# iris1997jiatong/I-DCCRN-VAE

Measured on AMD Instinct MI355X. Metric: 4s@16kHz utterances/sec fwd+SI-SNR, DCCRN-CL, 1/2/4/8 MI355X vs host CPU, higher is better.
Workload: dtype f32; 1 GPU; supervised DCCRN-CL forward(train=False) + final_ete_loss (weights 0/0/1); batch_per_gpu=64, utterance=4 s @ 16 kHz (64000 samples, 641 frames), parallelism=replicas x1, streams=1, input=resident in HBM

## Files before the change

i-dccrn-vae_amd/csrc/cgemm.hpp:

```cpp
#pragma once
#include "common.hpp"

#ifndef IDV_WAVES_PER_SIMD
#define IDV_WAVES_PER_SIMD 1
#endif

enum { IDV_CONV = 0, IDV_TCONV = 1, IDV_PW = 2 };

struct CgemmArgs {
    const float* x0;
    const float* x1;
    int C0, C1;
    int Fin, Fout;
    int J, Jp, Tp;
    int Jp1, x1_div;
    const float* wfrag;
    const float* bias;
    const float* slope;
    float* out;
    int M;
    int Mtiles;
    int cplx_rows;
    int Cout;
    int tshift;
    int t_valid;
    double* stats;
    int stats_rep;
    int ldo;
    int nB;
    int jtiles, ftiles, mblocks;
    int map_ft;
    long long lo_off0, lo_off1;
    void* out_img;
    long long out_lo_off;
};
#define IDV_IMG_ZSLOT (-8)

typedef __bf16 idv_bf16x2 __attribute__((ext_vector_type(2)));
__device__ __forceinline__ unsigned idv_pack_bf16(float a, float b) {
    idv_bf16x2 v = {(__bf16)a, (__bf16)b};
    return __builtin_bit_cast(unsigned, v);
}

template <int MODE, int FO_T>
struct CgemmGeom {
    static constexpr int KF = (MODE == IDV_PW) ? 1 : 5;
    static constexpr int FR = (MODE == IDV_CONV) ? 2 * FO_T + 3 : (MODE == IDV_TCONV ? FO_T + 2 : 1);
    static constexpr int ROWS = (MODE == IDV_TCONV) ? 2 * FO_T : FO_T;
};

struct CgemmFlatCols {
    static constexpr bool FLAT = true;
    __device__ __forceinline__ int in_col(const CgemmArgs&, int v) const { return v; }
    __device__ __forceinline__ void out_pos(const CgemmArgs& a, int v, int& b, int& tp) const {
        b = v / a.Tp;
        tp = v - b * a.Tp;
    }
    __device__ __forceinline__ void store(float* p, float y) const { *p = y; }
};
struct CgemmTimeChunkCols {
    static constexpr bool FLAT = false;
    int t0, steps;
    __device__ __forceinline__ int in_col(const CgemmArgs& a, int v) const {
        const int b = v / steps;
        return b * a.Tp + 1 + t0 + (v - b * steps);
    }
    __device__ __forceinline__ void out_pos(const CgemmArgs&, int v, int& b, int& tp) const {
        b = v / steps;
        tp = 1 + t0 + (v - b * steps);
    }
    __device__ __forceinline__ void store(float* p, float y) const { __hip_atomic_store(p, y, __ATOMIC_RELAXED, __HIP_MEMORY_SCOPE_AGENT); }
};

template <int MODE, int WM, int WN, int MT_W, int FO_T, int JC_W, int CCK, bool SWAP, bool STATS, bool VEC, class CM>
__device__ __forceinline__ void cgemm_tile(const CgemmArgs& a, float* smem, const int jt, const int ft, const int mblk, const CM cm) {
#define CGEMM_BODY_TILE_GIVEN
#include "cgemm_body.hpp"
#undef CGEMM_BODY_TILE_GIVEN
}

template <int MODE, int WM, int WN, int MT_W, int FO_T, int JC_W, int CCK, bool SWAP, bool STATS, bool VEC>
__global__ __launch_bounds__(WM* WN * 64, IDV_WAVES_PER_SIMD) void cgemm_kernel(const CgemmArgs a) {
    extern __shared__ __attribute__((aligned(16))) float smem[];
    using CM = CgemmFlatCols;
    const CM cm{};
#include "cgemm_body.hpp"
}
```

i-dccrn-vae_amd/csrc/cgemm_body.hpp:

```cpp
    using G = CgemmGeom<MODE, FO_T>;
    static_assert(CM::FLAT || (MODE == IDV_PW && SWAP && !VEC), "mapped columns: scalar staging of the point-wise SWAP form");
    constexpr int NT = WM * WN * 64;
    constexpr int KF = G::KF, FR = G::FR, ROWS = G::ROWS;
    constexpr int JT = 32 * JC_W * WN;
    constexpr int PS = VEC ? JT + 8 : JT + 2;
    constexpr int COL0 = VEC ? 4 : 1;
    constexpr int NE = CCK * FR * PS;
    constexpr int NLD = VEC ? 1 : (NE + NT - 1) / NT;
    constexpr int PS4 = PS / 4;
    constexpr int NV = CCK * FR * PS4;
    constexpr int NLD4 = VEC ? (NV + NT - 1) / NT : 1;
    static_assert(!VEC || NLD4 <= 8, "ok-mask holds 8 slots x 4 bits");
    constexpr int NCOL = ROWS * JC_W;
    constexpr int KSC = (MODE == IDV_PW) ? CCK / 2 : CCK * KF;
    static_assert(MODE != IDV_PW || (CCK % 2 == 0), "PW chunks are plane pairs");

    const int tid = threadIdx.x;
    const int lane = tid & 63;
    const int wave = __builtin_amdgcn_readfirstlane(tid >> 6);
    const int wm = wave / WN, wn = wave % WN;
#ifndef CGEMM_BODY_TILE_GIVEN

    const int MB = a.mblocks, FTn = a.ftiles;
    const int bid = blockIdx.x;
// ... 185 lines not shown

    constexpr int UNITS = (MODE == IDV_PW) ? CCK / 2 : CCK;
    const int bcol = wn * (JC_W * 32) + (lane & 31) + ((MODE == IDV_PW) ? COL0 : (lane >> 5) + COL0 + a.tshift);
    auto load_b = [&](const float* P, int u, float (&dst)[FR][JC_W]) {
#pragma unroll
        for (int fr = 0; fr < FR; ++fr)
#pragma unroll
            for (int jc = 0; jc < JC_W; ++jc) {
                if (MODE == IDV_PW)
                    dst[fr][jc] = P[(2 * u + (lane >> 5)) * PS + bcol + jc * 32];
                else
                    dst[fr][jc] = P[(u * FR + fr) * PS + bcol + jc * 32];
            }
    };

    stage_load(0);
    load_a(0, a_cur);
    stage_store(smem, 0);
#pragma unroll
    for (int ks = 0; ks < KSC; ++ks)
#pragma unroll
        for (int i = 0; i < MT_W; ++i) asm volatile("" : "+v"(a_cur[ks][i]));
    __syncthreads();

    for (int chunk = 0; chunk < nchunk; ++chunk) {
        const float* P = smem + (chunk & 1) * NE;
        const int nxt = (chunk + 1 < nchunk) ? chunk + 1 : chunk;
        float b_cur[FR][JC_W], b_nxt[FR][JC_W];
        load_b(P, 0, b_cur);
#pragma unroll
        for (int u = 0; u < UNITS; ++u) {
            if (u + 1 < UNITS) load_b(P, u + 1, b_nxt);
            __builtin_amdgcn_sched_barrier(0);
            if constexpr (CM::FLAT) {
                if (u == 0) {
                    stage_load(nxt);
                    load_a(nxt, a_nxt);
                }
            } else {
                constexpr int SPU = (2 * NLD + UNITS - 1) / UNITS;
#pragma unroll
                for (int q = 0; q < SPU; ++q)
                    if (u * SPU + q < NLD) stage_load_slot(nxt, u * SPU + q);
                static_assert(MODE != IDV_PW || KSC == UNITS, "one k-step per unit");
            }
            if (u == UNITS - 1) stage_store(smem + ((chunk + 1) & 1) * NE, nxt);
#pragma unroll
            for (int kf = 0; kf < KF; ++kf) {
                const int ks = (MODE == IDV_PW) ? u : u * KF + kf;
#pragma unroll
                for (int rt = 0; rt < ROWS; ++rt) {
                    int fr;
                    if (MODE == IDV_CONV) {
                        fr = 2 * rt + kf;
                    } else if (MODE == IDV_TCONV) {
                        if ((rt & 1) != (kf & 1)) continue;
                        fr = (rt >> 1) + 2 - (kf >> 1);
                    } else {
                        fr = 0;
                    }
#pragma unroll
                    for (int jc = 0; jc < JC_W; ++jc)
#pragma unroll
                        for (int i = 0; i < MT_W; ++i) {
                            if (SWAP)
                                acc[i][rt * JC_W + jc] = __builtin_amdgcn_mfma_f32_32x32x2f32(b_cur[fr][jc], a_cur[ks][i], acc[i][rt * JC_W + jc], 0, 0, 0);
                            else
                                acc[i][rt * JC_W + jc] = __builtin_amdgcn_mfma_f32_32x32x2f32(a_cur[ks][i], b_cur[fr][jc], acc[i][rt * JC_W + jc], 0, 0, 0);
                        }
                }
            }
            if constexpr (!CM::FLAT) load_a_ks(nxt, u, a_cur);
            if (u + 1 < UNITS) {
#pragma unroll
                for (int fr = 0; fr < FR; ++fr)
#pragma unroll
                    for (int jc = 0; jc < JC_W; ++jc) b_cur[fr][jc] = b_nxt[fr][jc];
            }
        }
        if constexpr (CM::FLAT) {
#pragma unroll
            for (int ks = 0; ks < KSC; ++ks)
#pragma unroll
                for (int i = 0; i < MT_W; ++i) a_cur[ks][i] = a_nxt[ks][i];
        }
        __syncthreads();
    }

    if (a.out_img && blockIdx.x == 0 && tid < 2) {
        unsigned short* z = (unsigned short*)a.out_img + IDV_IMG_ZSLOT * 8 + (tid ? a.out_lo_off : 0);
        *(uint4*)z = make_uint4(0u, 0u, 0u, 0u);
    }
    const float slope = a.slope ? *a.slope : 1.0f;
    const bool has_act = a.slope != nullptr;
    const int half = lane >> 5, l31 = lane & 31;

    if (!SWAP) {
#pragma unroll
        for (int i = 0; i < MT_W; ++i) {
            const int mt = mt0 + i;
            float bia[16];
#pragma unroll
            for (int r = 0; r < 16; ++r) {
                const int m = mt * 32 + (r & 3) + 8 * (r >> 2) + 4 * half;
                bia[r] = a.bias[m];
            }
            float st[STATS ? 8 : 1][5];
            if (STATS) {
#pragma unroll
                for (int q = 0; q < 8; ++q)
#pragma unroll
                    for (int s = 0; s < 5; ++s) st[q][s] = 0.f;
            }
// ... 96 lines not shown
```

i-dccrn-vae_amd/csrc/lstm.hip:

```cpp
#include "common.hpp"
#include "../../include/idccrn_hip.h"

namespace {

struct RecArgs {
    const float* g;
    long long g_run_z;
    long long g_run_s;
    int ldg;
    const float* whh;
    float* hout;
    int H, B, T;
    float* gsave;
    float* csave;
    void* kimg;
    long long kimg_lo;
    int Tp, Jp;
};

template <bool WREG>
__global__ __launch_bounds__(256, 1) void lstm_rec_kernel(const RecArgs a) {
    extern __shared__ __attribute__((aligned(16))) float sm[];
    const int H = WREG ? 128 : a.H;
    float* hT = sm;
// ... 570 lines not shown

}

static long long hp_floats(int H, int B, int Jp) {
    long long n = 4LL * H * Jp;
    if (idv_lstm_pers_supported(H, B)) {
        const long long m = (idv_lstm_pers_work_bytes(H, B) + 3) / 4;
        if (m > n) n = m;
    }
    if (idv_lstm_coop_f32_supported(H, B)) {
        const long long m = (idv_lstm_coop_f32_work_bytes(H, B) + 3) / 4;
        if (m > n) n = m;
    }
    if (idv_lstm_pers_f32_supported(H, B)) {
        const long long m = (idv_lstm_pers_f32_work_bytes(H, B) + 3) / 4;
        if (m > n) n = m;
    }
    if (idv_lstm_stack2_f32_supported(H, B)) {
        const long long m = (idv_lstm_stack2_f32_proj_work_bytes(H, B, Jp / B) + 3) / 4;
        if (m > n) n = m;
    }
    return (n + 63) / 64 * 64;
}

extern "C" long long idv_clstm_work_floats(int H, int B, int T, int Jp) {
    return 24LL * T * B * H + 4LL * B * H + hp_floats(H, B, Jp) + 4LL * H * Jp;
}
extern "C" long long idv_clstm_train_work_floats(int H, int B, int T, int Jp) {
    return 48LL * T * B * H + 4LL * B * H + hp_floats(H, B, Jp) + 4LL * H * Jp;
}

static int clstm_fwd_impl(const float* x, int K, const float* wih0, const float* bih0, const float* whh0,
                          const float* wih1, const float* bih1, const float* whh1, int H, int B, int T, int Tp, int Jp,
                          float* work, float* out, int flags, const void* wih1_bf16, const float* wih1_hh, int proj_c0, void* stream) {
    if (!x || !wih0 || !bih0 || !whh0 || !wih1 || !bih1 || !whh1 || !work || !out) return IDV_EINVAL;
    if (H <= 0 || (H % 16) || K <= 0 || (K & 1) || B <= 0 || T <= 0 || Tp < T + 1 || Jp < B * Tp) return IDV_EINVAL;
    if ((size_t)3 * H * 16 * sizeof(float) > 160 * 1024) return IDV_EINVAL;
    hipStream_t st = (hipStream_t)stream;
    const long long TB = (long long)T * B;
    const bool save = (flags & 4) != 0;
    if (save && (flags & 1) && H != 128 && ((flags & 8) || !idv_lstm_pers_supported(H, B))) return IDV_EINVAL;
    float* G = work;
    float* G1 = save ? work + 16 * TB * H : work;
    float* h0 = (save ? G1 : work) + 16 * TB * H;
    float* h1 = h0 + 4 * TB * H;
    float* c0 = save ? h1 + 4 * TB * H : nullptr;
    float* c1 = save ? c0 + 4 * TB * H : nullptr;
    float* cstate = (save ? c1 : h1) + 4 * TB * H;
    int rc;
    const bool stack2 = wih1_hh && !(flags & 1) && !(flags & 8) && idv_lstm_stack2_f32_supported(H, B) && 16LL * TB * H < 0xfffffe00LL;
    const bool fused = stack2 && !(flags & 2) && !(flags & 16) && idv_lstm_stack2_f32_proj_split(H, B, T, K, proj_c0, nullptr, nullptr);
    for (int z = 0; z < 2 && !(flags & 2) && !fused; ++z) {
        rc = idv_pw_gemm(x + (size_t)z * K * Jp, K, wih0, bih0, nullptr, G + (size_t)z * TB * 8 * H, 8 * H, B, Tp, Jp, T, 1,
                         8 * H, stream);
        if (rc) return rc;
    }
    const bool img1 = (flags & 1) && !(flags & 8) && wih1_bf16 && idv_lstm_pers_supported(H, B) &&
                      idv_lstm_proj_bf16_supported(H, H) && (4 * H) % 256 == 0;
    float* hp = cstate + 4LL * B * H;
    void* himg = (void*)(hp + hp_floats(H, B, Jp));
    const long long himg_lo = 4LL * (H / 8) * Jp;
    if (stack2) {
        if (fused)
            rc = idv_lstm_stack2_f32_proj(x, K, Tp, Jp, wih0, bih0, G, whh0, wih1_hh, whh1, bih1, h0, h1, H, B, T,
                                          (void*)(cstate + 4LL * B * H), save ? G1 : nullptr, c0, c1, proj_c0, stream);
        else
            rc = idv_lstm_stack2_f32(G, TB * 8 * H, 4LL * H, 8 * H, whh0, wih1_hh, whh1, bih1, h0, h1, H, B, T,
                                     (void*)(cstate + 4LL * B * H), save ? G1 : nullptr, c0, c1, stream);
        if (rc) return rc;
        hipLaunchKernelGGL(lstm_combine_kernel, dim3((T + 31) / 32, (H + 31) / 32, B), dim3(256), 0, st, h1, H, B, T, Tp, Jp, out);
        const long long ntail2 = 2LL * H * B * (Tp - 1 - T);
        if (ntail2 > 0)
            hipLaunchKernelGGL(zero_tail_kernel, dim3((unsigned)((ntail2 + 255) / 256 > 4096 ? 4096 : (ntail2 + 255) / 256)), dim3(256), 0,
                               st, out, 2 * H, B, T, Tp, Jp);
        return idv_launch_status();
    }
    RecArgs r0{G, TB * 8 * H, 4LL * H, 8 * H, whh0, h0, H, B, T, save ? G : nullptr, c0, img1 ? himg : nullptr, himg_lo, Tp, Jp};
    if ((rc = launch_rec(r0, cstate, flags, st))) return rc;
    const int KS = ((H + 7) / 8) * 4;
    dim3 ggrid((unsigned)((TB + 31) / 32), 4);
    if (img1) {
        if ((rc = idv_lstm_proj1_bf16x3(himg, himg_lo, wih1_bf16, bih1, G1, H, B, T, Tp, Jp, stream))) return rc;
    } else if (H == 128) {
        hipLaunchKernelGGL(gemm_rm_kernel<4>, ggrid, dim3(256), 0, st, h0, wih1, bih1, G1, H, TB, KS);
    } else if (H % 32 == 0) {
        hipLaunchKernelGGL(lstm_to_planar_kernel, dim3((T + 31) / 32, (H + 31) / 32, 4 * B), dim3(256), 0, st, h0, H, B, T, Tp, Jp, hp);
        if ((rc = idv_launch_status())) return rc;
        for (int run = 0; run < 4; ++run) {
            const int sset = run & 1;
            rc = idv_pw_gemm(hp + (size_t)run * H * Jp, H, wih1 + (size_t)sset * (4 * H / 32) * KS * 64, bih1 + sset * 4 * H, nullptr,
                             G1 + (size_t)run * TB * 4 * H, 4 * H, B, Tp, Jp, T, 1, 4 * H, stream);
            if (rc) return rc;
        }
    } else {
        const size_t smem = (size_t)32 * (H + 1) * sizeof(float);
        if (smem > 64 * 1024 &&
            hipFuncSetAttribute((const void*)gemm_rm_generic_kernel, hipFuncAttributeMaxDynamicSharedMemorySize, (int)smem) != hipSuccess)
            return IDV_ELAUNCH;
        hipLaunchKernelGGL(gemm_rm_generic_kernel, ggrid, dim3(256), smem, st, h0, wih1, bih1, G1, H, TB, KS);
    }
    if ((rc = idv_launch_status())) return rc;
    RecArgs r1{G1, 2 * TB * 4 * H, TB * 4 * H, 4 * H, whh1, h1, H, B, T, save ? G1 : nullptr, c1, nullptr, 0, Tp, Jp};
    if ((rc = launch_rec(r1, cstate, flags, st))) return rc;
    hipLaunchKernelGGL(lstm_combine_kernel, dim3((T + 31) / 32, (H + 31) / 32, B), dim3(256), 0, st, h1, H, B, T, Tp, Jp, out);
    const long long ntail = 2LL * H * B * (Tp - 1 - T);
    if (ntail > 0)
        hipLaunchKernelGGL(zero_tail_kernel, dim3((unsigned)((ntail + 255) / 256 > 4096 ? 4096 : (ntail + 255) / 256)), dim3(256), 0,
                           st, out, 2 * H, B, T, Tp, Jp);
    return idv_launch_status();
}

extern "C" int idv_clstm_fwd(const float* x, int K, const float* wih0, const float* bih0, const float* whh0,
                             const float* wih1, const float* bih1, const float* whh1, int H, int B, int T, int Tp, int Jp,
                             float* work, float* out, int flags, const void* wih1_bf16, void* stream) {
    return clstm_fwd_impl(x, K, wih0, bih0, whh0, wih1, bih1, whh1, H, B, T, Tp, Jp, work, out, flags, wih1_bf16, nullptr, -1, stream);
}

extern "C" int idv_clstm_fwd2(const float* x, int K, const float* wih0, const float* bih0, const float* whh0,
                              const float* wih1, const float* bih1, const float* whh1, const float* wih1_hh, int H, int B, int T,
                              int Tp, int Jp, float* work, float* out, int flags, const void* wih1_bf16, void* stream) {
    return clstm_fwd_impl(x, K, wih0, bih0, whh0, wih1, bih1, whh1, H, B, T, Tp, Jp, work, out, flags, wih1_bf16, wih1_hh, -1, stream);
}

extern "C" int idv_clstm_fwd3(const float* x, int K, const float* wih0, const float* bih0, const float* whh0,
                              const float* wih1, const float* bih1, const float* whh1, const float* wih1_hh, int H, int B, int T,
                              int Tp, int Jp, float* work, float* out, int flags, const void* wih1_bf16, int proj_c0, void* stream) {
    return clstm_fwd_impl(x, K, wih0, bih0, whh0, wih1, bih1, whh1, H, B, T, Tp, Jp, work, out, flags, wih1_bf16, wih1_hh, proj_c0, stream);
}
```

i-dccrn-vae_amd/csrc/lstm_proj_split.hpp:

```cpp
#pragma once

#if defined(__HIPCC__) || defined(__CUDACC__)
#define PROJ_HD __host__ __device__
#else
#define PROJ_HD
#endif

constexpr int PROJ_CH = 16;
constexpr int PROJ_STEP_NS = 3900;
constexpr int PROJ_TILE_NS_PER_K = 96;
constexpr int PROJ_TIE_PCT = 1;

struct ProjSplit {
    int nchunks;
    int gfull, glast;
    int c0;
    int P;
    long long nopen;
    long long ntiles;
};
struct ProjTile {
    int chunk, grp, z, mb;
    int t0, steps;
};

PROJ_HD inline int proj_chunk_steps(int T, int c) { return (c + 1) * PROJ_CH <= T ? PROJ_CH : T - c * PROJ_CH; }
PROJ_HD inline int proj_chunk_groups(int B, int T, int c) { return (proj_chunk_steps(T, c) * B + 63) / 64; }
PROJ_HD inline int proj_chunk_tiles(int B, int T, int c) { return 8 * proj_chunk_groups(B, T, c); }
PROJ_HD inline long long proj_tiles_before(const ProjSplit& s, int c) {
    return c < s.nchunks ? 8LL * s.gfull * c : 8LL * s.gfull * (s.nchunks - 1) + 8LL * s.glast;
}

PROJ_HD inline int proj_producers(const ProjSplit& s, int c0, int rec, int bound) {
    const long long room = (long long)bound - rec, rest = s.ntiles - proj_tiles_before(s, c0);
    return room <= 0 ? 0 : (int)(rest < room ? rest : room);
}

PROJ_HD inline long long proj_predict_ns(const ProjSplit& s, int B, int T, int K, int rec, int bound, int c0) {
    const long long tile_ns = (long long)PROJ_TILE_NS_PER_K * K;
    const long long nopen = proj_tiles_before(s, c0);
    const int P = proj_producers(s, c0, rec, bound);
    const long long W = c0 < s.nchunks ? rec + P : (bound > rec ? bound : rec);
    const long long open = (nopen + W - 1) / W * tile_ns;
// ... 10 lines not shown

PROJ_HD inline ProjSplit proj_split(int B, int T, int K, int rec, int bound, int force_c0) {
    ProjSplit s;
    s.nchunks = (T + PROJ_CH - 1) / PROJ_CH;
    s.glast = proj_chunk_groups(B, T, s.nchunks - 1);
    s.gfull = s.nchunks > 1 ? (PROJ_CH * B + 63) / 64 : s.glast;
    s.ntiles = 8LL * s.gfull * (s.nchunks - 1) + 8LL * s.glast;
    s.c0 = s.nchunks;
    s.P = 0;
    s.nopen = s.ntiles;
    if (bound <= rec) return s;
    if (force_c0 >= 0) {
        s.c0 = force_c0 < s.nchunks ? force_c0 : s.nchunks;
        s.P = proj_producers(s, s.c0, rec, bound);
        if (s.P == 0) s.P = 1;
    } else {
        long long best = proj_predict_ns(s, B, T, K, rec, bound, 0);
        for (int c = 1; c < s.nchunks; ++c) {
            const long long p = proj_predict_ns(s, B, T, K, rec, bound, c);
            if (p < best) best = p;
        }
        const long long lim = best + best * PROJ_TIE_PCT / 100;
        if (proj_predict_ns(s, B, T, K, rec, bound, s.nchunks) > lim) {
            int c0 = 0;
            while (proj_predict_ns(s, B, T, K, rec, bound, c0) > lim) ++c0;
            s.c0 = c0;
            s.P = proj_producers(s, c0, rec, bound);
        }
    }
    s.nopen = proj_tiles_before(s, s.c0);
    return s;
}

struct ProjWalk {
    long long i, stride, end;
};
PROJ_HD inline ProjWalk proj_walk(const ProjSplit& s, int wg, int nwg) {
    ProjWalk w;
    w.i = wg;
    w.stride = nwg;
    w.end = s.nopen;
    return w;
}
PROJ_HD inline bool proj_walk_tile(const ProjSplit& s, ProjWalk& w, int pid) {
    if (w.i >= w.end) {
        if (pid < 0 || w.end == s.ntiles) return false;
        w.i = s.nopen + pid;
        w.stride = s.P;
        w.end = s.ntiles;
        if (w.i >= w.end) return false;
    }
    return true;
}

PROJ_HD inline ProjTile proj_tile(const ProjSplit& s, int T, long long i) {
    ProjTile t;
    const long long per = 8LL * s.gfull;
    t.chunk = (int)(i / per);
    if (t.chunk >= s.nchunks - 1) t.chunk = s.nchunks - 1;
    const int r = (int)(i - per * t.chunk);
    t.grp = r >> 3;
    t.z = (r >> 2) & 1;
    t.mb = r & 3;
    t.t0 = t.chunk * PROJ_CH;
    t.steps = proj_chunk_steps(T, t.chunk);
    return t;
}
```

i-dccrn-vae_amd/csrc/lstm_stack2_f32.hip:

```cpp
#include <cstdlib>
#include "cgemm.hpp"
#include "coop.hpp"
#include "lstm_proj_split.hpp"
#include "../../include/idccrn_hip.h"

namespace idv_stack2 {

typedef int v4i __attribute__((ext_vector_type(4)));

struct Args {
    const float* x;
    const float* wih0;
    const float* bih0;
    int K, Tp, Jp;
    unsigned g_bytes;
    ProjSplit ps;
    const float* g;
    long long g_run_z, g_run_s;
    int ldg;
    const float* whh0;
    const float* wih1;
    const float* whh1;
    const float* bias1;
    float* h0;
    unsigned h0_bytes;
    float* hout;
    float* gsave1;
    float* csave0;
    float* csave1;
    float* hx;
    unsigned hx_bytes;
    CoopSync cs;
    int B, T, Bpad, tiles;
};

constexpr int H = 128, NSL = 4, UPW = 32;
constexpr int MAX_GROUPS = 64, MAX_REP = 8;
constexpr int SYNC_BYTES = idv_coop_sync_bytes(2 * MAX_GROUPS, MAX_REP);
constexpr int PROJ_CCK = 32;
constexpr int RED_FLOATS = 4 * 8 * 4 * 64;
constexpr int proj_sync_bytes(int T) { return idv_coop_sync_bytes(2 * MAX_GROUPS + (T + PROJ_CH - 1) / PROJ_CH, MAX_REP); }

template <bool PROJ>
__global__ __launch_bounds__(256, 1) void lstm_stack2_f32_kernel(const Args a) {
    extern __shared__ __attribute__((aligned(16))) float red[];
    __shared__ int abort_sh;
    __shared__ unsigned seen0_sh;
    __shared__ __attribute__((aligned(16))) float stage[16][UPW];
    const __amdgpu_buffer_rsrc_t hxr = __builtin_amdgcn_make_buffer_rsrc((void*)a.hx, 0, a.hx_bytes, 0x00020000);
    const __amdgpu_buffer_rsrc_t h0r = __builtin_amdgcn_make_buffer_rsrc((void*)a.h0, 0, a.h0_bytes, 0x00020000);
    const int tid = threadIdx.x, lane = tid & 63;
    const int wave = __builtin_amdgcn_readfirstlane(tid >> 6);
    const int nrec = 2 * NSL * 4 * a.tiles;
    const bool producer = PROJ && (int)blockIdx.x >= nrec;
    const int rid = producer ? 0 : (int)blockIdx.x;
    const int layer = PROJ ? (rid >> 2) & 1 : blockIdx.x >> 2, sl = blockIdx.x & 3;
    const int run = PROJ ? (rid >> 3) & 3 : blockIdx.y, tile = PROJ ? rid >> 5 : blockIdx.z;
    const int z = run >> 1, s = run & 1;
    const int col = lane & 15, rq = lane >> 4;
    const int b0 = tile * 16;
    unsigned* abortf = idv_coop_abort_flag(a.cs);
    const int groups = 4 * a.tiles, grp = run * a.tiles + tile;
    unsigned* cnt0 = idv_coop_counter(a.cs, 0 * groups + grp);
    unsigned* cnt1 = idv_coop_counter(a.cs, 1 * groups + grp);
    unsigned* mine = layer ? cnt1 : cnt0;
    const size_t TB = (size_t)a.T * a.B, TBH = TB * H;
    const unsigned hx_layer = (unsigned)layer * 2u * 4u * (unsigned)a.Bpad * (unsigned)H * 4u;
    const unsigned hx_par = 4u * (unsigned)a.Bpad * (unsigned)H * 4u;

    const __amdgpu_buffer_rsrc_t gr = __builtin_amdgcn_make_buffer_rsrc((void*)a.g, 0, PROJ ? a.g_bytes : 0u, 0x00020000);
    if constexpr (PROJ) {
        if (idv_coop_withheld(a.cs)) return;
        for (ProjWalk w = proj_walk(a.ps, (int)blockIdx.x, (int)gridDim.x);
             proj_walk_tile(a.ps, w, producer ? (int)blockIdx.x - nrec : -1); w.i += w.stride) {
            const ProjTile pt = proj_tile(a.ps, a.T, w.i);
            CgemmArgs ca{};
            ca.x0 = a.x + (size_t)pt.z * a.K * a.Jp;
            ca.C0 = a.K / 2;
            ca.Fin = 1; ca.Fout = 1;
            ca.J = pt.steps * a.B; ca.Jp = a.Jp; ca.Tp = a.Tp;
            ca.wfrag = a.wih0; ca.bias = a.bih0;
            ca.out = const_cast<float*>(a.g) + (size_t)pt.z * a.g_run_z;
            ca.M = 8 * H; ca.Mtiles = 8 * H / 32; ca.Cout = 8 * H;
            ca.t_valid = a.T; ca.ldo = a.ldg; ca.nB = a.B;
            cgemm_tile<IDV_PW, 4, 1, 2, 1, 2, PROJ_CCK, true, false, false>(ca, red + RED_FLOATS, pt.grp, 0, pt.mb,
                                                                            CgemmTimeChunkCols{pt.t0, pt.steps});
            asm volatile("s_waitcnt vmcnt(0)" ::: "memory");
            __syncthreads();
            idv_coop_arrive(a.cs, idv_coop_counter(a.cs, 2 * groups + pt.chunk), tid);
        }
        if (producer) return;
    }

    float breg[8][8], ireg[8][8];
    {
        const float* wb = (layer ? a.whh1 : a.whh0) + (size_t)s * 4 * H * H;
        const float* wi = a.wih1 + (size_t)s * 4 * H * H;
#pragma unroll
        for (int t8 = 0; t8 < 8; ++t8) {
            const int ctile = (2 * sl + (t8 >> 2)) * 4 + (t8 & 3);
#pragma unroll
            for (int j = 0; j < 8; ++j) {
                const int k = 32 * wave + 8 * rq + j;
                const size_t e = ((size_t)ctile * (H / 4) + (k >> 2)) * 64 + (k & 3) * 16 + col;
                breg[t8][j] = wb[e];
                ireg[t8][j] = layer ? wi[e] : 0.f;
            }
// ... 10 lines not shown
    for (int ub = 0; ub < 2; ++ub)
#pragma unroll
        for (int gg = 0; gg < 4; ++gg) gb[ub][gg] = layer ? a.bias1[(size_t)s * 4 * H + (2 * sl + ub) * 64 + 16 * gg + col] : 0.f;
    const float* g = a.g + z * a.g_run_z + s * a.g_run_s;
    float* gsv = !a.csave0 ? nullptr : (layer ? a.gsave1 + (size_t)run * TB * 4 * H : const_cast<float*>(g));
    const int gld = layer ? 4 * H : a.ldg;
    float* csv = layer ? a.csave1 : a.csave0;

    bool aborted = false;
    if (tid == 0) { abort_sh = 0; seen0_sh = 0; }
    if (idv_coop_withheld(a.cs)) return;
    __syncthreads();

    auto input_known = [&](int tt) -> bool { return seen0_sh >= (unsigned)(tt + 1) * (unsigned)NSL; };
    auto input_load = [&](int tt, f32x4& a0, f32x4& a1) {
        const unsigned off = (unsigned)((((size_t)run * TB + (size_t)tt * a.B + lrow) * H + 32 * wave + 8 * rq) * 4u);
        a0 = __builtin_bit_cast(f32x4, __builtin_amdgcn_raw_buffer_load_b128(h0r, off, 0, 16));
        a1 = __builtin_bit_cast(f32x4, __builtin_amdgcn_raw_buffer_load_b128(h0r, off + 16u, 0, 16));
    };
    auto input_late = [&](int tt, f32x4& a0, f32x4& a1) -> bool {
        if (tid == 0) idv_coop_wait(idv_coop_replica(a.cs, cnt0, sl), (unsigned)(tt + 1) * (unsigned)NSL, abortf, &abort_sh, &seen0_sh);
        __syncthreads();
        if (abort_sh) return false;
        input_load(tt, a0, a1);
        return true;
    };
    f32x4 cur0 = {0.f, 0.f, 0.f, 0.f}, cur1 = {0.f, 0.f, 0.f, 0.f};
    if (layer && !input_late(0, cur0, cur1)) aborted = true;

    for (int t = 0; t < a.T && !aborted; ++t) {
        float gpre[2][4];
        if (layer == 0) {
            if constexpr (PROJ) {
                if (t % PROJ_CH == 0) {
                    const int c = t / PROJ_CH;
                    if (tid == 0)
                        idv_coop_wait(idv_coop_replica(a.cs, idv_coop_counter(a.cs, 2 * groups + c), sl),
                                      (unsigned)proj_chunk_tiles(a.B, a.T, c), abortf, &abort_sh);
                    __syncthreads();
                    if (abort_sh) { aborted = true; break; }
                }
                const unsigned off = (unsigned)(((size_t)z * a.g_run_z + (size_t)s * a.g_run_s + ((size_t)t * a.B + bclamp) * a.ldg +
                                                 (2 * sl) * 64 + col) * 4u);
#pragma unroll
                for (int ub = 0; ub < 2; ++ub)
#pragma unroll
                    for (int gg = 0; gg < 4; ++gg)
                        gpre[ub][gg] = __builtin_bit_cast(float, __builtin_amdgcn_raw_buffer_load_b32(gr, off + (ub * 64 + 16 * gg) * 4u, 0, 16));
            } else {
                const float* gp = g + ((size_t)t * a.B + bclamp) * a.ldg + (2 * sl) * 64 + col;
#pragma unroll
                for (int ub = 0; ub < 2; ++ub)
#pragma unroll
                    for (int gg = 0; gg < 4; ++gg) gpre[ub][gg] = gp[ub * 64 + 16 * gg];
            }
        } else {
#pragma unroll
            for (int ub = 0; ub < 2; ++ub)
#pragma unroll
                for (int gg = 0; gg < 4; ++gg) gpre[ub][gg] = gb[ub][gg];
        }
        f32x4 acc[8];
#pragma unroll
        for (int t8 = 0; t8 < 8; ++t8)
#pragma unroll
            for (int r = 0; r < 4; ++r) acc[t8][r] = 0.f;
        auto input_mfma = [&]() {
// ... 120 lines not shown
    if ((gsave1 != nullptr) != (csave0 != nullptr) || (csave0 != nullptr) != (csave1 != nullptr)) return IDV_EINVAL;
    if ((reinterpret_cast<uintptr_t>(work) & 15) || (reinterpret_cast<uintptr_t>(h0) & 15) || (reinterpret_cast<uintptr_t>(hout) & 15))
        return IDV_EINVAL;
    const long long h0_bytes = 4LL * T * B * H * 4;
    if (h0_bytes >= 0xfffffe00LL) return IDV_EINVAL;
    hipStream_t st = (hipStream_t)stream;
    const int tiles = (B + 15) / 16;
    const long long Bpad = 16LL * tiles;
    Args a{};
    a.g = g; a.g_run_z = g_run_z; a.g_run_s = g_run_s; a.ldg = ldg;
    a.whh0 = whh0; a.wih1 = wih1_hh; a.whh1 = whh1; a.bias1 = bias1;
    a.h0 = h0; a.h0_bytes = (unsigned)h0_bytes; a.hout = hout;
    a.gsave1 = gsave1; a.csave0 = csave0; a.csave1 = csave1;
    a.hx = (float*)((char*)work + SYNC_BYTES);
    a.hx_bytes = (unsigned)(2LL * 2 * 4 * Bpad * H * 4);
    a.cs.nrep = 4;
    a.B = B; a.T = T; a.Bpad = (int)Bpad; a.tiles = tiles;
    const size_t smem = 84 * 1024;
    return idv_coop_launch(lstm_stack2_f32_kernel<false>, dim3(2 * NSL, 4, tiles), smem, st, work, SYNC_BYTES, a);
}

extern "C" int idv_lstm_stack2_f32_proj_split(int H, int B, int T, int K, int force_c0, int* c0, int* P) {
    static const bool on = [] { const char* e = getenv("IDV_LSTM_PROJ_OVERLAP"); return !e || e[0] != '0'; }();
    if (c0) *c0 = 0;
    if (P) *P = 0;
    if (!on || T <= 0 || K <= 0 || (K & 1) || !idv_lstm_stack2_f32_supported(H, B)) return 0;
    if (64LL * T * B * H >= 0xfffffe00LL) return 0;
    const ProjSplit ps = proj_split(B, T, K, 2 * 4 * 4 * ((B + 15) / 16), idv_coop_max_workgroups(), force_c0);
    if (c0) *c0 = ps.c0;
    if (P) *P = ps.P;
    return ps.P > 0;
}

extern "C" long long idv_lstm_stack2_f32_proj_work_bytes(int H, int B, int Tmax) {
    const long long Bpad = (B + 15) / 16 * 16;
    return idv_stack2::proj_sync_bytes(Tmax < 1 ? 1 : Tmax) + 2LL * 2 * 4 * Bpad * H * 4;
}

extern "C" int idv_lstm_stack2_f32_proj(const float* x, int K, int Tp, int Jp, const float* wih0, const float* bih0, float* g,
                                        const float* whh0, const float* wih1_hh, const float* whh1, const float* bias1, float* h0,
                                        float* hout, int H, int B, int T, void* work, float* gsave1, float* csave0, float* csave1,
                                        int force_c0, void* stream) {
    using namespace idv_stack2;
    if (!x || !wih0 || !bih0 || !g || !whh0 || !wih1_hh || !whh1 || !bias1 || !h0 || !hout || !work || T <= 0 || Tp < T + 1 ||
        (long long)Jp < (long long)B * Tp || !idv_lstm_stack2_f32_proj_split(H, B, T, K, force_c0, nullptr, nullptr))
        return IDV_EINVAL;
    if ((gsave1 != nullptr) != (csave0 != nullptr) || (csave0 != nullptr) != (csave1 != nullptr)) return IDV_EINVAL;
    if ((reinterpret_cast<uintptr_t>(work) & 15) || (reinterpret_cast<uintptr_t>(h0) & 15) || (reinterpret_cast<uintptr_t>(hout) & 15) ||
        (reinterpret_cast<uintptr_t>(g) & 3))
        return IDV_EINVAL;
    const long long TB = (long long)T * B;
    const int tiles = (B + 15) / 16;
    const long long Bpad = 16LL * tiles;
    const int sync_bytes = proj_sync_bytes(T);
    Args a{};
    a.x = x; a.wih0 = wih0; a.bih0 = bih0; a.K = K; a.Tp = Tp; a.Jp = Jp;
    a.g_bytes = (unsigned)(64LL * TB * H);
    a.ps = proj_split(B, T, K, 2 * NSL * 4 * tiles, idv_coop_max_workgroups(), force_c0);
    a.g = g; a.g_run_z = TB * 8 * H; a.g_run_s = 4LL * H; a.ldg = 8 * H;
    a.whh0 = whh0; a.wih1 = wih1_hh; a.whh1 = whh1; a.bias1 = bias1;
    a.h0 = h0; a.h0_bytes = (unsigned)(16LL * TB * H); a.hout = hout;
    a.gsave1 = gsave1; a.csave0 = csave0; a.csave1 = csave1;
    a.hx = (float*)((char*)work + sync_bytes);
    a.hx_bytes = (unsigned)(2LL * 2 * 4 * Bpad * H * 4);
    a.cs.nrep = 4;
    a.B = B; a.T = T; a.Bpad = (int)Bpad; a.tiles = tiles;
    const size_t smem = 84 * 1024;
    return idv_coop_launch(lstm_stack2_f32_kernel<true>, dim3(2 * NSL * 4 * tiles + a.ps.P), smem, (hipStream_t)stream, work,
                           sync_bytes, a);
}
```

include/idccrn_hip.h:

```cpp
#ifndef IDCCRN_HIP_H
#define IDCCRN_HIP_H

#ifdef __cplusplus
extern "C" {
#endif

#define IDV_ABI_VERSION 9
#define IDV_SLACK_FLOATS 256

int idv_abi_version(void);

int idv_coop_last_status(int clear);
int idv_coop_max_workgroups(void);


int idv_cconv_cck(int cin_used);
int idv_cconv_config(int transposed, int cin_used, int Cout, int Fin);

int idv_cbn_fold(const float* moments, const float* gamma_rr, const float* gamma_ri, const float* gamma_ii,
                 const float* beta_r, const float* beta_i, int C, float* fold, void* stream);

int idv_pack_cconv(const float* w_re, const float* w_im, const float* b_re, const float* b_im, const float* fold,
                   int Cout, int Cin_total, int Cin_used, int transposed, float* wfrag, float* bias_out, void* stream);

// ... 99 lines not shown
                          int B, int T, int Tp, int Jp, void* stream);
int idv_lstm_coop_f32_supported(int H, int B);
long long idv_lstm_coop_f32_work_bytes(int H, int B);
int idv_lstm_rec_coop_f32(const float* g, long long g_run_z, long long g_run_s, int ldg, const float* whh_frag, float* hout, int H,
                          int B, int T, void* work, float* gsave, float* csave, void* stream);
int idv_lstm_pers_f32_supported(int H, int B);
long long idv_lstm_pers_f32_work_bytes(int H, int B);
int idv_lstm_rec_pers_f32(const float* g, long long g_run_z, long long g_run_s, int ldg, const float* whh_frag, float* hout, int H,
                          int B, int T, void* work, float* gsave, float* csave, void* stream);
void idv_lstm_pers_set_profile(unsigned long long* prof_cycles);
long long idv_clstm_train_work_floats(int H, int B, int T, int Jp);
int idv_clstm_fwd(const float* x, int K, const float* wih0, const float* bih0, const float* whh0, const float* wih1,
                  const float* bih1, const float* whh1, int H, int B, int T, int Tp, int Jp, float* work, float* out,
                  int flags, const void* wih1_bf16, void* stream);

int idv_lstm_stack2_f32_supported(int H, int B);
long long idv_lstm_stack2_f32_work_bytes(int H, int B);
int idv_lstm_stack2_f32(const float* g, long long g_run_z, long long g_run_s, int ldg, const float* whh0, const float* wih1_hh,
                        const float* whh1, const float* bias1, float* h0, float* hout, int H, int B, int T, void* work,
                        float* gsave1, float* csave0, float* csave1, void* stream);
int idv_clstm_fwd2(const float* x, int K, const float* wih0, const float* bih0, const float* whh0, const float* wih1,
                   const float* bih1, const float* whh1, const float* wih1_hh, int H, int B, int T, int Tp, int Jp, float* work,
                   float* out, int flags, const void* wih1_bf16, void* stream);

int idv_lstm_stack2_f32_proj_split(int H, int B, int T, int K, int force_c0, int* c0, int* P);
long long idv_lstm_stack2_f32_proj_work_bytes(int H, int B, int Tmax);
int idv_lstm_stack2_f32_proj(const float* x, int K, int Tp, int Jp, const float* wih0, const float* bih0, float* g,
                             const float* whh0, const float* wih1_hh, const float* whh1, const float* bias1, float* h0,
                             float* hout, int H, int B, int T, void* work, float* gsave1, float* csave0, float* csave1,
                             int force_c0, void* stream);
int idv_clstm_fwd3(const float* x, int K, const float* wih0, const float* bih0, const float* whh0, const float* wih1,
                   const float* bih1, const float* whh1, const float* wih1_hh, int H, int B, int T, int Tp, int Jp, float* work,
                   float* out, int flags, const void* wih1_bf16, int proj_c0, void* stream);

long long idv_lstm_ih_bf16_bytes(int H, int K);
int idv_lstm_proj_bf16_supported(int H, int K);
int idv_pack_lstm_ih_bf16(const float* w_ih_re, const float* w_ih_im, int H, int K, void* wfrag, void* stream);
int idv_planar_to_kimage(const float* x, int nvalid, int nplanes, int J, int Jp, void* img, long long lo_off_elems, void* stream);
int idv_pw_bf16_coltile(int M, int B, int Tp);
int idv_pw_bf16x3_rows(const void* ximg, long long lo_off_slots, int K, const void* wfrag_bf16, const float* bias, float* out_rows,
                       int M, int ldo, int B, int T, int Tp, int Jp, void* stream);
long long idv_pw_bf16_wfrag_bytes(int M, int K);
int idv_pack_pw_bf16(const float* w, int M, int K, void* wfrag, void* stream);
int idv_pw_bf16x3(const void* ximg, long long lo_off_slots, int K, const void* wfrag_bf16, const float* bias, float* out, int M,
                  int B, int Tp, int Jp, int t_valid, void* stream);
int idv_stft_frames_kimage(const float* x, int B, int L, int n_fft, int win, int hop, int T, void* img, long long lo_off_elems,
                           int Tp, int Jp, void* stream);
int idv_lstm_proj_bf16x3(const void* ximg, long long lo_off_slots, int K, const void* wfrag_bf16, const float* bias, float* G,
                         int H, int B, int T, int Tp, int Jp, void* stream);

int idv_reparam(const float* lat, int Hl, int off_miu, int off_ls, int off_dl, int zdim, const float* eps_r,
                const float* eps_i, int ns, int B, int T, int Tp, int Jp, float* z, int Jpz, void* stream);


int idv_sisnr(const float* source, int src_ld, int src_div, const float* est, int est_ld, int B, int L, double* work,
              float* out, void* stream);
int idv_sisdr(const float* ref, int ref_ld, const float* est, int est_ld, int B, int L, double* work, float* out, void* stream);
int idv_mean_over_samples(const float* x, int ns, int B, int L, float* out, void* stream);
int idv_recon_loss(const float* pred_c, const float* ori, long long sb, long long sf, long long st, long long sr,
                   int ori_div, int B, int F, int T, double* work, float* out, void* stream);
int idv_ckl(const float* q1, int H1, int Jp1, int o1_miu, int o1_ls, int o1_dl, const float* q2, int H2, int Jp2,
            int o2_miu, int o2_ls, int o2_dl, int zdim, float eps, int B, int T, int Tp, double* work, float* out,
            void* stream);
int idv_msd(const float* a, int Ca, int ca0, int JpA, const float* b, int Cb, int cb0, int JpB, int C, int F, int B, int Tp,
            int t_valid, double* work, float* out, void* stream);
long long idv_mi_work_floats(int B, int ns, int T, int zdim);
// ... 375 lines not shown
```

Baseline: 1100 utterances/sec.

## Precompute leading LSTM input-projection chunks in a full-width front kernel

Result: no change. 1104 utterances/sec, median of 6 (+0.4%).

```diff
diff --git a/i-dccrn-vae_amd/csrc/cgemm.hpp b/i-dccrn-vae_amd/csrc/cgemm.hpp
--- a/i-dccrn-vae_amd/csrc/cgemm.hpp
+++ b/i-dccrn-vae_amd/csrc/cgemm.hpp
@@ -50,7 +50,7 @@
 };
 
 struct CgemmFlatCols {
-    static constexpr bool FLAT = true;
+    static constexpr bool FLAT = true, SPREAD = false;
     __device__ __forceinline__ int in_col(const CgemmArgs&, int v) const { return v; }
     __device__ __forceinline__ void out_pos(const CgemmArgs& a, int v, int& b, int& tp) const {
         b = v / a.Tp;
@@ -59,7 +59,7 @@
     __device__ __forceinline__ void store(float* p, float y) const { *p = y; }
 };
 struct CgemmTimeChunkCols {
-    static constexpr bool FLAT = false;
+    static constexpr bool FLAT = false, SPREAD = true;
     int t0, steps;
     __device__ __forceinline__ int in_col(const CgemmArgs& a, int v) const {
         const int b = v / steps;
diff --git a/i-dccrn-vae_amd/csrc/cgemm_body.hpp b/i-dccrn-vae_amd/csrc/cgemm_body.hpp
--- a/i-dccrn-vae_amd/csrc/cgemm_body.hpp
+++ b/i-dccrn-vae_amd/csrc/cgemm_body.hpp
@@ -241,7 +241,7 @@
         for (int u = 0; u < UNITS; ++u) {
             if (u + 1 < UNITS) load_b(P, u + 1, b_nxt);
             __builtin_amdgcn_sched_barrier(0);
-            if constexpr (CM::FLAT) {
+            if constexpr (!CM::SPREAD) {
                 if (u == 0) {
                     stage_load(nxt);
                     load_a(nxt, a_nxt);
@@ -279,7 +279,7 @@
                         }
                 }
             }
-            if constexpr (!CM::FLAT) load_a_ks(nxt, u, a_cur);
+            if constexpr (CM::SPREAD) load_a_ks(nxt, u, a_cur);
             if (u + 1 < UNITS) {
 #pragma unroll
                 for (int fr = 0; fr < FR; ++fr)
@@ -287,7 +287,7 @@
                     for (int jc = 0; jc < JC_W; ++jc) b_cur[fr][jc] = b_nxt[fr][jc];
             }
         }
-        if constexpr (CM::FLAT) {
+        if constexpr (!CM::SPREAD) {
 #pragma unroll
             for (int ks = 0; ks < KSC; ++ks)
 #pragma unroll
diff --git a/i-dccrn-vae_amd/csrc/lstm.hip b/i-dccrn-vae_amd/csrc/lstm.hip
--- a/i-dccrn-vae_amd/csrc/lstm.hip
+++ b/i-dccrn-vae_amd/csrc/lstm.hip
@@ -626,7 +626,7 @@
 
 static int clstm_fwd_impl(const float* x, int K, const float* wih0, const float* bih0, const float* whh0,
                           const float* wih1, const float* bih1, const float* whh1, int H, int B, int T, int Tp, int Jp,
-                          float* work, float* out, int flags, const void* wih1_bf16, const float* wih1_hh, int proj_c0, void* stream) {
+                          float* work, float* out, int flags, const void* wih1_bf16, const float* wih1_hh, int proj_c0, int front_c0, void* stream) {
     if (!x || !wih0 || !bih0 || !whh0 || !wih1 || !bih1 || !whh1 || !work || !out) return IDV_EINVAL;
     if (H <= 0 || (H % 16) || K <= 0 || (K & 1) || B <= 0 || T <= 0 || Tp < T + 1 || Jp < B * Tp) return IDV_EINVAL;
     if ((size_t)3 * H * 16 * sizeof(float) > 160 * 1024) return IDV_EINVAL;
@@ -643,7 +643,9 @@
     float* cstate = (save ? c1 : h1) + 4 * TB * H;
     int rc;
     const bool stack2 = wih1_hh && !(flags & 1) && !(flags & 8) && idv_lstm_stack2_f32_supported(H, B) && 16LL * TB * H < 0xfffffe00LL;
-    const bool fused = stack2 && !(flags & 2) && !(flags & 16) && idv_lstm_stack2_f32_proj_split(H, B, T, K, proj_c0, nullptr, nullptr);
+    const bool front = stack2 && !(flags & 2) && !(flags & 16) && proj_c0 < 0 && front_c0 >= -1 &&
+                       idv_lstm_stack2_f32_front_split(H, B, T, K, front_c0, nullptr, nullptr);
+    const bool fused = front || (stack2 && !(flags & 2) && !(flags & 16) && idv_lstm_stack2_f32_proj_split(H, B, T, K, proj_c0, nullptr, nullptr));
     for (int z = 0; z < 2 && !(flags & 2) && !fused; ++z) {
         rc = idv_pw_gemm(x + (size_t)z * K * Jp, K, wih0, bih0, nullptr, G + (size_t)z * TB * 8 * H, 8 * H, B, Tp, Jp, T, 1,
                          8 * H, stream);
@@ -655,7 +657,10 @@
     void* himg = (void*)(hp + hp_floats(H, B, Jp));
     const long long himg_lo = 4LL * (H / 8) * Jp;
     if (stack2) {
-        if (fused)
+        if (front)
+            rc = idv_lstm_stack2_f32_front(x, K, Tp, Jp, wih0, bih0, G, whh0, wih1_hh, whh1, bih1, h0, h1, H, B, T,
+                                           (void*)(cstate + 4LL * B * H), save ? G1 : nullptr, c0, c1, front_c0, stream);
+        else if (fused)
             rc = idv_lstm_stack2_f32_proj(x, K, Tp, Jp, wih0, bih0, G, whh0, wih1_hh, whh1, bih1, h0, h1, H, B, T,
                                           (void*)(cstate + 4LL * B * H), save ? G1 : nullptr, c0, c1, proj_c0, stream);
         else
@@ -707,17 +712,24 @@
 extern "C" int idv_clstm_fwd(const float* x, int K, const float* wih0, const float* bih0, const float* whh0,
                              const float* wih1, const float* bih1, const float* whh1, int H, int B, int T, int Tp, int Jp,
                              float* work, float* out, int flags, const void* wih1_bf16, void* stream) {
-    return clstm_fwd_impl(x, K, wih0, bih0, whh0, wih1, bih1, whh1, H, B, T, Tp, Jp, work, out, flags, wih1_bf16, nullptr, -1, stream);
+    return clstm_fwd_impl(x, K, wih0, bih0, whh0, wih1, bih1, whh1, H, B, T, Tp, Jp, work, out, flags, wih1_bf16, nullptr, -1, -1, stream);
 }
 
 extern "C" int idv_clstm_fwd2(const float* x, int K, const float* wih0, const float* bih0, const float* whh0,
                               const float* wih1, const float* bih1, const float* whh1, const float* wih1_hh, int H, int B, int T,
                               int Tp, int Jp, float* work, float* out, int flags, const void* wih1_bf16, void* stream) {
-    return clstm_fwd_impl(x, K, wih0, bih0, whh0, wih1, bih1, whh1, H, B, T, Tp, Jp, work, out, flags, wih1_bf16, wih1_hh, -1, stream);
+    return clstm_fwd_impl(x, K, wih0, bih0, whh0, wih1, bih1, whh1, H, B, T, Tp, Jp, work, out, flags, wih1_bf16, wih1_hh, -1, -1, stream);
 }
 
 extern "C" int idv_clstm_fwd3(const float* x, int K, const float* wih0, const float* bih0, const float* whh0,
                               const float* wih1, const float* bih1, const float* whh1, const float* wih1_hh, int H, int B, int T,
                               int Tp, int Jp, float* work, float* out, int flags, const void* wih1_bf16, int proj_c0, void* stream) {
-    return clstm_fwd_impl(x, K, wih0, bih0, whh0, wih1, bih1, whh1, H, B, T, Tp, Jp, work, out, flags, wih1_bf16, wih1_hh, proj_c0, stream);
-}
+    return clstm_fwd_impl(x, K, wih0, bih0, whh0, wih1, bih1, whh1, H, B, T, Tp, Jp, work, out, flags, wih1_bf16, wih1_hh, proj_c0, -1, stream);
+}
+
+extern "C" int idv_clstm_fwd4(const float* x, int K, const float* wih0, const float* bih0, const float* whh0,
+                              const float* wih1, const float* bih1, const float* whh1, const float* wih1_hh, int H, int B, int T,
+                              int Tp, int Jp, float* work, float* out, int flags, const void* wih1_bf16, int proj_c0, int front_c0,
+                              void* stream) {
+    return clstm_fwd_impl(x, K, wih0, bih0, whh0, wih1, bih1, whh1, H, B, T, Tp, Jp, work, out, flags, wih1_bf16, wih1_hh, proj_c0, front_c0, stream);
+}
diff --git a/i-dccrn-vae_amd/csrc/lstm_proj_front.hip b/i-dccrn-vae_amd/csrc/lstm_proj_front.hip
--- /dev/null
+++ b/i-dccrn-vae_amd/csrc/lstm_proj_front.hip
@@ -0,0 +1,61 @@
+#include "cgemm.hpp"
+#include "lstm_proj_split.hpp"
+#include "../../include/idccrn_hip.h"
+
+namespace {
+
+struct TimeChunkPlainCols {
+    static constexpr bool FLAT = false, SPREAD = false;
+    int t0, steps;
+    __device__ __forceinline__ int in_col(const CgemmArgs& a, int v) const {
+        const int b = v / steps;
+        return b * a.Tp + 1 + t0 + (v - b * steps);
+    }
+    __device__ __forceinline__ void out_pos(const CgemmArgs&, int v, int& b, int& tp) const {
+        b = v / steps;
+        tp = 1 + t0 + (v - b * steps);
+    }
+    __device__ __forceinline__ void store(float* p, float y) const { *p = y; }
+};
+
+struct FrontArgs {
+    const float* x;
+    const float* wih0;
+    const float* bih0;
+    float* g;
+    int K, Tp, Jp, B, T, M;
+    ProjSplit ps;
+};
+
+constexpr int CCK = 8, JT = 64;
+constexpr int NE = CCK * (JT + 2);
+
+__global__ __launch_bounds__(256, 3) void lstm_proj_front_kernel(const FrontArgs a) {
+    __shared__ __attribute__((aligned(16))) float smem[2 * NE];
+    const long long bid = blockIdx.x;
+    const long long i = (bid & ~31LL) + ((bid & 7) << 2) + ((bid >> 3) & 3);
+    if (i >= a.ps.nopen) return;
+    const ProjTile pt = proj_tile(a.ps, a.T, i);
+    CgemmArgs ca{};
+    ca.x0 = a.x + (size_t)pt.z * a.K * a.Jp;
+    ca.C0 = a.K / 2;
+    ca.Fin = 1; ca.Fout = 1;
+    ca.J = pt.steps * a.B; ca.Jp = a.Jp; ca.Tp = a.Tp;
+    ca.wfrag = a.wih0; ca.bias = a.bih0;
+    ca.out = a.g + (size_t)pt.z * a.T * a.B * a.M;
+    ca.M = a.M; ca.Mtiles = a.M / 32; ca.Cout = a.M;
+    ca.t_valid = a.T; ca.ldo = a.M; ca.nB = a.B;
+    cgemm_tile<IDV_PW, 4, 1, 2, 1, 2, CCK, true, false, false>(ca, smem, pt.grp, 0, pt.mb, TimeChunkPlainCols{pt.t0, pt.steps});
+}
+
+}
+
+int idv_launch_lstm_proj_front(const float* x, int K, int Tp, int Jp, const float* wih0, const float* bih0, float* g, int H, int B,
+                               int T, const ProjSplit& ps, hipStream_t st) {
+    if (ps.nopen <= 0 || ps.nopen > ps.ntiles || (ps.nopen & 7)) return IDV_EINVAL;
+    FrontArgs a{x, wih0, bih0, g, K, Tp, Jp, B, T, 8 * H, ps};
+    const long long nblk = (ps.nopen + 31) / 32 * 32;
+    if (nblk > 0x7fffffffLL) return IDV_EINVAL;
+    hipLaunchKernelGGL(lstm_proj_front_kernel, dim3((unsigned)nblk), dim3(256), 0, st, a);
+    return idv_launch_status();
+}
diff --git a/i-dccrn-vae_amd/csrc/lstm_proj_split.hpp b/i-dccrn-vae_amd/csrc/lstm_proj_split.hpp
--- a/i-dccrn-vae_amd/csrc/lstm_proj_split.hpp
+++ b/i-dccrn-vae_amd/csrc/lstm_proj_split.hpp
@@ -9,6 +9,7 @@
 constexpr int PROJ_CH = 16;
 constexpr int PROJ_STEP_NS = 3900;
 constexpr int PROJ_TILE_NS_PER_K = 96;
+constexpr int PROJ_FRONT_TILE_NS_PER_K = 89;
 constexpr int PROJ_TIE_PCT = 1;
 
 struct ProjSplit {
@@ -85,6 +86,47 @@
     return s;
 }
 
+PROJ_HD inline long long proj_front_predict_ns(const ProjSplit& s, int B, int T, int K, int rec, int bound, int cus, int c0) {
+    const long long tile_ns = (long long)PROJ_TILE_NS_PER_K * K, front_tile_ns = (long long)PROJ_FRONT_TILE_NS_PER_K * K;
+    const long long nfront = proj_tiles_before(s, c0);
+    const int P = proj_producers(s, c0, rec, bound);
+    const long long front = (nfront * front_tile_ns + cus - 1) / cus;
+    long long t = front;
+    for (int c = 0; c < s.nchunks; ++c) {
+        if (c >= c0) {
+            const long long ready = front + (proj_tiles_before(s, c + 1) - nfront + P - 1) / P * tile_ns;
+            if (ready > t) t = ready;
+        }
+        t += (long long)proj_chunk_steps(T, c) * PROJ_STEP_NS;
+    }
+    return t;
+}
+
+PROJ_HD inline ProjSplit proj_front_split(int B, int T, int K, int rec, int bound, int cus, int force_c0) {
+    ProjSplit s = proj_split(B, T, K, rec, bound, -1);
+    const long long fused = proj_predict_ns(s, B, T, K, rec, bound, s.c0), hoisted = proj_predict_ns(s, B, T, K, rec, bound, s.nchunks);
+    const long long old = fused < hoisted ? fused : hoisted;
+    s.c0 = s.nchunks;
+    s.P = 0;
+    s.nopen = s.ntiles;
+    if (bound <= rec || s.nchunks < 2 || cus < 1) return s;
+    int c0 = 1;
+    if (force_c0 >= 0) {
+        c0 = force_c0 < 1 ? 1 : (force_c0 < s.nchunks ? force_c0 : s.nchunks - 1);
+    } else {
+        long long best = proj_front_predict_ns(s, B, T, K, rec, bound, cus, 1);
+        for (int c = 2; c < s.nchunks; ++c) {
+            const long long p = proj_front_predict_ns(s, B, T, K, rec, bound, cus, c);
+            if (p < best) { best = p; c0 = c; }
+        }
+        if (best + best * PROJ_TIE_PCT / 100 >= old) return s;
+    }
+    s.c0 = c0;
+    s.P = proj_producers(s, c0, rec, bound);
+    s.nopen = proj_tiles_before(s, c0);
+    return s;
+}
+
 struct ProjWalk {
     long long i, stride, end;
 };
@@ -93,6 +135,13 @@
     w.i = wg;
     w.stride = nwg;
     w.end = s.nopen;
+    return w;
+}
+PROJ_HD inline ProjWalk proj_walk_front(const ProjSplit& s, int pid) {
+    ProjWalk w;
+    w.i = pid < 0 ? s.ntiles : s.nopen + pid;
+    w.stride = s.P;
+    w.end = s.ntiles;
     return w;
 }
 PROJ_HD inline bool proj_walk_tile(const ProjSplit& s, ProjWalk& w, int pid) {
diff --git a/i-dccrn-vae_amd/csrc/lstm_stack2_f32.hip b/i-dccrn-vae_amd/csrc/lstm_stack2_f32.hip
--- a/i-dccrn-vae_amd/csrc/lstm_stack2_f32.hip
+++ b/i-dccrn-vae_amd/csrc/lstm_stack2_f32.hip
@@ -15,6 +15,7 @@
     int K, Tp, Jp;
     unsigned g_bytes;
     ProjSplit ps;
+    int front;
     const float* g;
     long long g_run_z, g_run_s;
     int ldg;
@@ -71,8 +72,9 @@
     const __amdgpu_buffer_rsrc_t gr = __builtin_amdgcn_make_buffer_rsrc((void*)a.g, 0, PROJ ? a.g_bytes : 0u, 0x00020000);
     if constexpr (PROJ) {
         if (idv_coop_withheld(a.cs)) return;
-        for (ProjWalk w = proj_walk(a.ps, (int)blockIdx.x, (int)gridDim.x);
-             proj_walk_tile(a.ps, w, producer ? (int)blockIdx.x - nrec : -1); w.i += w.stride) {
+        const int pid = producer ? (int)blockIdx.x - nrec : -1;
+        for (ProjWalk w = a.front ? proj_walk_front(a.ps, pid) : proj_walk(a.ps, (int)blockIdx.x, (int)gridDim.x);
+             proj_walk_tile(a.ps, w, pid); w.i += w.stride) {
             const ProjTile pt = proj_tile(a.ps, a.T, w.i);
             CgemmArgs ca{};
             ca.x0 = a.x + (size_t)pt.z * a.K * a.Jp;
@@ -149,7 +151,7 @@
         float gpre[2][4];
         if (layer == 0) {
             if constexpr (PROJ) {
-                if (t % PROJ_CH == 0) {
+                if (t % PROJ_CH == 0 && t / PROJ_CH >= a.front) {
                     const int c = t / PROJ_CH;
                     if (tid == 0)
                         idv_coop_wait(idv_coop_replica(a.cs, idv_coop_counter(a.cs, 2 * groups + c), sl),
@@ -336,18 +338,44 @@
     return ps.P > 0;
 }
 
+int idv_launch_lstm_proj_front(const float* x, int K, int Tp, int Jp, const float* wih0, const float* bih0, float* g, int H, int B,
+                               int T, const ProjSplit& ps, hipStream_t st);
+
+static int device_cus() {
+    int dev = 0, n = 0;
+    if (hipGetDevice(&dev) != hipSuccess || hipDeviceGetAttribute(&n, hipDeviceAttributeMultiprocessorCount, dev) != hipSuccess || n <= 0) {
+        (void)hipGetLastError();
+        return 256;
+    }
+    return n;
+}
+
+extern "C" int idv_lstm_stack2_f32_front_split(int H, int B, int T, int K, int force_c0, int* c0, int* P) {
+    static const bool on = [] { const char* e = getenv("IDV_LSTM_PROJ_OVERLAP"); return !e || e[0] != '0'; }();
+    if (c0) *c0 = 0;
+    if (P) *P = 0;
+    if (!on || T <= 0 || K <= 0 || (K & 1) || !idv_lstm_stack2_f32_supported(H, B)) return 0;
+    if (64LL * T * B * H >= 0xfffffe00LL) return 0;
+    const ProjSplit ps = proj_front_split(B, T, K, 2 * 4 * 4 * ((B + 15) / 16), idv_coop_max_workgroups(), device_cus(), force_c0);
+    if (ps.P <= 0) return 0;
+    if (c0) *c0 = ps.c0;
+    if (P) *P = ps.P;
+    return 1;
+}
+
 extern "C" long long idv_lstm_stack2_f32_proj_work_bytes(int H, int B, int Tmax) {
     const long long Bpad = (B + 15) / 16 * 16;
     return idv_stack2::proj_sync_bytes(Tmax < 1 ? 1 : Tmax) + 2LL * 2 * 4 * Bpad * H * 4;
 }
 
-extern "C" int idv_lstm_stack2_f32_proj(const float* x, int K, int Tp, int Jp, const float* wih0, const float* bih0, float* g,
-                                        const float* whh0, const float* wih1_hh, const float* whh1, const float* bias1, float* h0,
-                                        float* hout, int H, int B, int T, void* work, float* gsave1, float* csave0, float* csave1,
-                                        int force_c0, void* stream) {
+static int stack2_proj_launch(const float* x, int K, int Tp, int Jp, const float* wih0, const float* bih0, float* g,
+                              const float* whh0, const float* wih1_hh, const float* whh1, const float* bias1, float* h0,
+                              float* hout, int H, int B, int T, void* work, float* gsave1, float* csave0, float* csave1,
+                              int force_c0, bool front, void* stream) {
     using namespace idv_stack2;
     if (!x || !wih0 || !bih0 || !g || !whh0 || !wih1_hh || !whh1 || !bias1 || !h0 || !hout || !work || T <= 0 || Tp < T + 1 ||
-        (long long)Jp < (long long)B * Tp || !idv_lstm_stack2_f32_proj_split(H, B, T, K, force_c0, nullptr, nullptr))
+        (long long)Jp < (long long)B * Tp ||
+        !(front ? idv_lstm_stack2_f32_front_split : idv_lstm_stack2_f32_proj_split)(H, B, T, K, force_c0, nullptr, nullptr))
         return IDV_EINVAL;
     if ((gsave1 != nullptr) != (csave0 != nullptr) || (csave0 != nullptr) != (csave1 != nullptr)) return IDV_EINVAL;
     if ((reinterpret_cast<uintptr_t>(work) & 15) || (reinterpret_cast<uintptr_t>(h0) & 15) || (reinterpret_cast<uintptr_t>(hout) & 15) ||
@@ -360,7 +388,13 @@
     Args a{};
     a.x = x; a.wih0 = wih0; a.bih0 = bih0; a.K = K; a.Tp = Tp; a.Jp = Jp;
     a.g_bytes = (unsigned)(64LL * TB * H);
-    a.ps = proj_split(B, T, K, 2 * NSL * 4 * tiles, idv_coop_max_workgroups(), force_c0);
+    if (front) {
+        a.ps = proj_front_split(B, T, K, 2 * NSL * 4 * tiles, idv_coop_max_workgroups(), device_cus(), force_c0);
+        a.front = a.ps.c0;
+        if (int rc = idv_launch_lstm_proj_front(x, K, Tp, Jp, wih0, bih0, g, H, B, T, a.ps, (hipStream_t)stream)) return rc;
+    } else {
+        a.ps = proj_split(B, T, K, 2 * NSL * 4 * tiles, idv_coop_max_workgroups(), force_c0);
+    }
     a.g = g; a.g_run_z = TB * 8 * H; a.g_run_s = 4LL * H; a.ldg = 8 * H;
     a.whh0 = whh0; a.wih1 = wih1_hh; a.whh1 = whh1; a.bias1 = bias1;
     a.h0 = h0; a.h0_bytes = (unsigned)(16LL * TB * H); a.hout = hout;
@@ -373,3 +407,19 @@
     return idv_coop_launch(lstm_stack2_f32_kernel<true>, dim3(2 * NSL * 4 * tiles + a.ps.P), smem, (hipStream_t)stream, work,
                            sync_bytes, a);
 }
+
+extern "C" int idv_lstm_stack2_f32_proj(const float* x, int K, int Tp, int Jp, const float* wih0, const float* bih0, float* g,
+                                        const float* whh0, const float* wih1_hh, const float* whh1, const float* bias1, float* h0,
+                                        float* hout, int H, int B, int T, void* work, float* gsave1, float* csave0, float* csave1,
+                                        int force_c0, void* stream) {
+    return stack2_proj_launch(x, K, Tp, Jp, wih0, bih0, g, whh0, wih1_hh, whh1, bias1, h0, hout, H, B, T, work, gsave1, csave0, csave1,
+                              force_c0, false, stream);
+}
+
+extern "C" int idv_lstm_stack2_f32_front(const float* x, int K, int Tp, int Jp, const float* wih0, const float* bih0, float* g,
+                                         const float* whh0, const float* wih1_hh, const float* whh1, const float* bias1, float* h0,
+                                         float* hout, int H, int B, int T, void* work, float* gsave1, float* csave0, float* csave1,
+                                         int force_c0, void* stream) {
+    return stack2_proj_launch(x, K, Tp, Jp, wih0, bih0, g, whh0, wih1_hh, whh1, bias1, h0, hout, H, B, T, work, gsave1, csave0, csave1,
+                              force_c0, true, stream);
+}
diff --git a/include/idccrn_hip.h b/include/idccrn_hip.h
--- a/include/idccrn_hip.h
+++ b/include/idccrn_hip.h
@@ -155,6 +155,14 @@
 int idv_clstm_fwd3(const float* x, int K, const float* wih0, const float* bih0, const float* whh0, const float* wih1,
                    const float* bih1, const float* whh1, const float* wih1_hh, int H, int B, int T, int Tp, int Jp, float* work,
                    float* out, int flags, const void* wih1_bf16, int proj_c0, void* stream);
+int idv_lstm_stack2_f32_front_split(int H, int B, int T, int K, int force_c0, int* c0, int* P);
+int idv_lstm_stack2_f32_front(const float* x, int K, int Tp, int Jp, const float* wih0, const float* bih0, float* g,
+                              const float* whh0, const float* wih1_hh, const float* whh1, const float* bias1, float* h0,
+                              float* hout, int H, int B, int T, void* work, float* gsave1, float* csave0, float* csave1,
+                              int force_c0, void* stream);
+int idv_clstm_fwd4(const float* x, int K, const float* wih0, const float* bih0, const float* whh0, const float* wih1,
+                   const float* bih1, const float* whh1, const float* wih1_hh, int H, int B, int T, int Tp, int Jp, float* work,
+                   float* out, int flags, const void* wih1_bf16, int proj_c0, int front_c0, void* stream);
 
 long long idv_lstm_ih_bf16_bytes(int H, int K);
 int idv_lstm_proj_bf16_supported(int H, int K);
```
